# huggingface/diffusers

Measured on AMD Instinct MI355X. Metric: images/sec @ SDXL-base 1024x1024 50-step EulerDiscrete CFG bf16, higher is better.
Workload: dtype bf16; 1 GPU; SDXL-base-1.0 U-Net (2567 M params) x 50 EulerDiscrete steps, CFG 5.0 (batch 2), 128x128 latents + AutoencoderKL decode to 1024x1024; 1 prompt per GPU; global_batch=1, parallelism=dp1 (independent prompts, replicas), denoise_steps=50, output_type=pt, hip_graph=True, output_finite=True, rccl_ranks=1, tuned_live=0, cpu_binding=none

## Files before the change

### diffusers_amd/_lib.py

```python
from __future__ import annotations

import ctypes as C
import threading
from pathlib import Path

_PKG = Path(__file__).resolve().parent
LIB_PATH = _PKG / "_C" / "libdiffusers_amd.so"

DA_OK = 0
ERRORS = {1: "DA_ERR_INVALID", 2: "DA_ERR_LAUNCH", 3: "DA_ERR_UNSUPPORTED"}
ACT_NONE, ACT_GEGLU, ACT_GELU_TANH, ACT_SILU, ACT_GELU_ERF, ACT_QUICK_GELU, ACT_GEGLU_TANH = 0, 1, 2, 3, 4, 5, 6
ACT_RELU = 7
(TILE_AUTO, TILE_128x128, TILE_64x128, TILE_128x64, TILE_64x64, TILE_256x128, TILE_128x256, TILE_256x256,
 TILE_128x128_W8, TILE_K2_128x128, TILE_K2_128x80, TILE_K2_128x160, TILE_K2_80x128, TILE_K2_128x64,
 TILE_K1_128x320, TILE_K1_256x128, TILE_K1_128x256, TILE_K1_256x160, TILE_K1_256x256, TILE_K1_256x320,
 TILE_K3_256x256, TILE_K3_256x320) = range(22)
TILE_NAMES = ("auto", "128x128", "64x128", "128x64", "64x64", "256x128", "128x256", "256x256", "128x128w8",
              "k2:128x128", "k2:128x80", "k2:128x160", "k2:80x128", "k2:128x64",
              "k1:128x320", "k1:256x128", "k1:128x256", "k1:256x160", "k1:256x256", "k1:256x320",
              "k3:256x256", "k3:256x320")
FIRST_K2_TILE = TILE_K2_128x128
STAGE_REGISTER, STAGE_LDS_DIRECT, STAGE_LDS_DIRECT3, STAGE_LDS_DIRECT4, STAGE_LDS_DIRECT6, STAGE_LDS_DIRECT8 = range(6)
STAGE_PINGPONG, STAGE_PINGPONG3 = 6, 7
RING_SLOTS = (2, 2, 3, 4, 6, 8)
# ... 14 lines not shown
        ("M", C.c_int), ("N", C.c_int), ("K", C.c_int),
        ("lda", C.c_int), ("ldw", C.c_int), ("ldc", C.c_int), ("ldr", C.c_int), ("ld_rowvec", C.c_int),
        ("ld_gate", C.c_int),
        ("rows_per_batch", C.c_int),
        ("alpha", C.c_float), ("out_scale", C.c_float),
        ("act", C.c_int), ("out_f32", C.c_int), ("conv", C.c_int),
        ("Hin", C.c_int), ("Win", C.c_int), ("C1", C.c_int), ("C2", C.c_int),
        ("Hout", C.c_int), ("Wout", C.c_int), ("stride", C.c_int), ("up", C.c_int), ("pad", C.c_int),
        ("tile", C.c_int), ("staging", C.c_int), ("gate_f32", C.c_int),
        ("split_k", C.c_int), ("workspace", C.c_void_p), ("sync_flags", C.c_void_p), ("workspace_bytes", C.c_longlong),
        ("stats_out", C.c_void_p), ("stats_ld", C.c_int), ("ln_stats", C.c_void_p), ("ln_stats_ld", C.c_int),
        ("ln_parts", C.c_int), ("ln_s", C.c_void_p), ("ln_c", C.c_void_p), ("ln_eps", C.c_float), ("k_valid", C.c_int),
        ("prefetch", C.c_void_p), ("prefetch_bytes", C.c_longlong),
        ("vt", C.c_void_p), ("vt_col0", C.c_int), ("ld_vt", C.c_longlong),
        ("xa_k", C.c_void_p), ("xa_vt", C.c_void_p), ("xa_skv", C.c_int), ("xa_skv_alloc", C.c_int), ("xa_k_ld", C.c_int),
        ("xa_vt_ld", C.c_longlong), ("xa_scale", C.c_float),
    ]


class AttentionParams(C.Structure):
    _fields_ = [
        ("q", C.c_void_p), ("k", C.c_void_p), ("vt", C.c_void_p), ("out", C.c_void_p),
        ("B", C.c_int), ("H", C.c_int), ("Sq", C.c_int), ("Skv", C.c_int), ("Skv_alloc", C.c_int), ("D", C.c_int),
        ("q_batch_stride", C.c_longlong), ("k_batch_stride", C.c_longlong),
        ("vt_batch_stride", C.c_longlong), ("o_batch_stride", C.c_longlong),
        ("q_row_stride", C.c_int), ("k_row_stride", C.c_int), ("vt_ld", C.c_int), ("o_row_stride", C.c_int),
        ("scale", C.c_float), ("ring_slots", C.c_int),
        ("bias", C.c_void_p), ("bias_batch_stride", C.c_longlong), ("bias_head_stride", C.c_longlong),
        ("bias_row_stride", C.c_int), ("bias_f32", C.c_int), ("causal", C.c_int), ("q_block", C.c_int), ("pv_delay", C.c_int),
        ("algo", C.c_int),
        ("split_ws", C.c_void_p), ("split_ws_bytes", C.c_longlong), ("kv_split", C.c_int),
# ... 138 lines not shown
```

### diffusers_amd/autoencoder_kl.py

```python
from __future__ import annotations

from dataclasses import dataclass
from typing import Dict, Optional

import torch

from . import ops
from .config_utils import check_to
from .loading import PretrainedMixin
from . import _lib as L
from .layers import Downsample2D, GroupNorm, ResnetBlock2D, Upsample2D, Weights
from .unet_2d_condition import FrozenConfig

bf16 = torch.bfloat16


@dataclass
class DecoderOutput:
    sample: torch.Tensor


_DEFAULTS = dict(
    in_channels=3, out_channels=3, down_block_types=("DownEncoderBlock2D",), up_block_types=("UpDecoderBlock2D",),
    block_out_channels=(64,), layers_per_block=1, act_fn="silu", latent_channels=4, norm_num_groups=32, sample_size=32,
# ... 239 lines not shown
        self.conv_in_w = ops.pack_conv_weight(ci)
        self.conv_in_b = w.get("decoder.conv_in.bias")

        self.mid_res0 = ResnetBlock2D(w, "decoder.mid_block.resnets.0", groups, eps)
        self.mid_attn = VaeAttention(w, "decoder.mid_block.attentions.0", groups, eps) \
            if c.mid_block_add_attention else None
        self.mid_res1 = ResnetBlock2D(w, "decoder.mid_block.resnets.1", groups, eps)

        self.up = []
        n = len(boc)
        for i in range(n):
            pre = f"decoder.up_blocks.{i}"
            stage = {"resnets": [ResnetBlock2D(w, f"{pre}.resnets.{j}", groups, eps)
                                 for j in range(c.layers_per_block + 1)], "up": None}
            if i != n - 1:
                stage["up"] = Upsample2D(w, f"{pre}.upsamplers.0")
            self.up.append(stage)
        self.conv_norm_out = GroupNorm(w, "decoder.conv_norm_out", groups, eps)
        self.conv_out_w = ops.pack_conv_weight(w.get("decoder.conv_out.weight"))
        self.conv_out_b = w.get("decoder.conv_out.bias")
        self.encoder = _Encoder(w, c, groups, eps) if w.has("encoder.conv_in.weight") else None
        if strict:
            extra = [k for k in w.unused() if k.startswith(("decoder.", "post_quant_conv.", "encoder.", "quant_conv."))]
            if extra:
                raise RuntimeError(f"unexpected VAE keys: {extra[:8]}")
        self._built = True
        return self

    def to(self, *args, **kwargs):
        return check_to(self, args, kwargs)

# ... 58 lines not shown
```

### diffusers_amd/csrc/gemm.hip

```cpp
#include "gemm_kernel.cuh"
#include "gemm2_shared.cuh"

namespace da_gemm {
int dispatch_conv(const da_gemm_params& p, int tile, int staging, hipStream_t s);
}
namespace da_gemm2 {
int dispatch_lin(const da_gemm_params& p, int tile, int staging, hipStream_t s);
int dispatch_conv(const da_gemm_params& p, int tile, int staging, hipStream_t s);
}
namespace da_gemm3 {
int dispatch_lin(const da_gemm_params& p, int tile, int staging, hipStream_t s);
}
namespace da_c64 {
int launch(const da_gemm_params& p, hipStream_t s);
}

namespace {

struct TileShape {
  int bm, bn, waves;
};
constexpr TileShape kTiles[] = {{0, 0, 0},      {128, 128, 4}, {64, 128, 4},  {128, 64, 4}, {64, 64, 4},
                                {256, 128, 8},  {128, 256, 8}, {256, 256, 8}, {128, 128, 8},
                                {128, 128, 8},  {128, 80, 8},  {128, 160, 8}, {80, 128, 8}, {128, 64, 8},
                                {128, 320, 8},  {256, 128, 8}, {128, 256, 8}, {256, 160, 8}, {256, 256, 8}, {256, 320, 8},
                                {256, 256, 8},  {256, 320, 8}};
static_assert(sizeof(kTiles) / sizeof(kTiles[0]) == DA_TILE_COUNT, "kTiles / DA_TILE_* mismatch");
inline bool is_k3(int tile) { return tile == DA_TILE_K3_256x256 || tile == DA_TILE_K3_256x320; }
inline bool is_k2(int tile) { return tile >= DA_TILE_K2_128x128 && !is_k3(tile); }
constexpr int kNumTiles = sizeof(kTiles) / sizeof(kTiles[0]);

int pick_tile(const da_gemm_params& p) {
  auto nblk = [&](int t) {
    return (long)((p.M + kTiles[t].bm - 1) / kTiles[t].bm) * ((p.N + kTiles[t].bn - 1) / kTiles[t].bn);
  };
  const bool geglu = (p.act == DA_ACT_GEGLU || p.act == DA_ACT_GEGLU_TANH);
  const bool narrow = !geglu && ((p.N & 127) != 0) && ((p.N % 128) <= 64);
  if (narrow) return (nblk(DA_TILE_128x64) >= 200) ? DA_TILE_128x64 : DA_TILE_64x64;
  if (nblk(DA_TILE_256x128) >= 480) return DA_TILE_256x128;
  if (nblk(DA_TILE_128x128) >= 128) return DA_TILE_128x128;
  if (nblk(DA_TILE_64x128) >= 128 || geglu) return DA_TILE_64x128;
  return DA_TILE_64x64;
}

int validate_conv(const da_gemm_params& p) {
  if (p.C1 <= 0 || (p.C1 & 63) || (p.C2 & 63) || p.C2 < 0) return DA_ERR_UNSUPPORTED;
  if (p.conv != 1 && p.conv != 3) return DA_ERR_UNSUPPORTED;
  if (p.K != p.conv * p.conv * (p.C1 + p.C2)) return DA_ERR_INVALID;
  if (p.stride != 1 && p.stride != 2) return DA_ERR_UNSUPPORTED;
  if (p.up != 0 && p.up != 1) return DA_ERR_INVALID;
  if (p.Hin <= 0 || p.Win <= 0 || p.Hout <= 0 || p.Wout <= 0) return DA_ERR_INVALID;
  if (p.M % (p.Hout * p.Wout)) return DA_ERR_INVALID;
  return DA_OK;
}

int validate(da_gemm_params& p) {
  if (p.M <= 0 || p.N <= 0 || p.K <= 0) return DA_ERR_INVALID;
  if ((p.K & 63) || (p.N & 3) || (p.ldc & 3)) return DA_ERR_UNSUPPORTED;
  if (!p.A || !p.W || !p.C) return DA_ERR_INVALID;
  if (p.residual && (p.ldr & 3)) return DA_ERR_UNSUPPORTED;
  if (p.rowvec && (p.rows_per_batch <= 0 || (p.ld_rowvec & 3))) return DA_ERR_INVALID;
  if (p.gate && (p.rows_per_batch <= 0 || (p.ld_gate & 3))) return DA_ERR_INVALID;
  if (p.gate_f32 < 0 || p.gate_f32 > 2) return DA_ERR_INVALID;
  if (p.alpha == 0.0f) p.alpha = 1.0f;
  if (p.out_scale == 0.0f) p.out_scale = 1.0f;
  if (p.conv) {
    const int v = validate_conv(p);
    if (v != DA_OK) return v;
    if (p.C2 > 0 && !p.A2) return DA_ERR_INVALID;
  } else {
    if ((p.lda & 7) || (p.ldw & 7)) return DA_ERR_UNSUPPORTED;
  }
  if ((p.act == DA_ACT_GEGLU || p.act == DA_ACT_GEGLU_TANH) &&
      ((p.N & 127) || p.out_f32 || p.residual || p.rowvec || p.gate || p.bias_rows))
    return DA_ERR_UNSUPPORTED;
  if (p.act < 0 || p.act > DA_ACT_RELU) return DA_ERR_INVALID;
  if (p.gate && p.gate_f32 == 2 && p.conv == 3) return DA_ERR_UNSUPPORTED;
  if (p.split_k < 0 || p.split_k > DA_SPLITK_MAX) return DA_ERR_INVALID;
  if (p.split_k > 1 && (p.stats_out || p.ln_stats)) return DA_ERR_UNSUPPORTED;
  if (p.k_valid < 0 || (p.k_valid > 0 && (p.k_valid > (p.conv ? p.C1 : p.K) || (p.conv && p.C2 != 0)))) return DA_ERR_INVALID;
// ... 4 lines not shown
    return DA_ERR_INVALID;
  return DA_OK;
}

int stats_parts(const da_gemm_params& p, int tile) {
  if (is_k2(tile)) {
    const int band = (tile == DA_TILE_K2_128x80 || tile == DA_TILE_K2_128x160) ? 80 : 0;
    return band ? (p.N + band - 1) / band : 0;
  }
  return (p.N + kTiles[tile].bn - 1) / kTiles[tile].bn;
}

bool tile_ok(const da_gemm_params& p, int tile) {
  if (tile <= 0 || tile >= kNumTiles) return false;
  if (p.act == DA_ACT_RELU) return false;
  if (p.gate && p.gate_f32 == 2 && (is_k2(tile) || is_k3(tile))) return false;
  if (is_k3(tile)) {
    if (p.conv || p.split_k > 1 || p.stats_out || (p.ln_stats && tile != DA_TILE_K3_256x320) || p.vt || p.xa_k) return false;
    if (tile == DA_TILE_K3_256x320)
      return (p.act == DA_ACT_GEGLU || p.act == DA_ACT_GEGLU_TANH) && (p.M % 256) == 0 && (p.N % 320) == 0 && !(p.ldc & 7) &&
             !((size_t)p.C & 15);
    return true;
  }
  if (is_k2(tile)) {
    const bool geglu = (p.act == DA_ACT_GEGLU || p.act == DA_ACT_GEGLU_TANH);
    const bool geglu_ok = tile == DA_TILE_K2_128x128 || tile == DA_TILE_K1_256x128 || tile == DA_TILE_K1_128x256 ||
                          tile == DA_TILE_K1_256x256 || tile == DA_TILE_K1_256x320 || (tile == DA_TILE_K1_128x320 && !p.conv);
    const bool lnf_lin = tile == DA_TILE_K2_128x80 || tile == DA_TILE_K2_128x160;
    const bool lnf_cons = lnf_lin || tile == DA_TILE_K1_128x256 || tile == DA_TILE_K1_256x128;
    if (p.xa_k) return !p.conv && p.split_k <= 1 && !geglu && !p.stats_out && !p.vt && tile == DA_TILE_K2_128x128;
// ... 160 lines not shown
```

### diffusers_amd/csrc/gemm2_kernel.cuh

```cuda
#pragma once
#include <cstdlib>
#include <type_traits>

#include "common.cuh"
#include "diffusers_amd.h"
#include "gemm2_shared.cuh"

namespace da_gemm2 {


#if defined(DA_GEMM2_TRACE)
__device__ unsigned long long* g_da2_trace;
#define DA2_TRACE(i) tr_[i] = __builtin_readcyclecounter()
#else
#define DA2_TRACE(i) ((void)0)
#endif



template <int KG, int WM, int WN, int MT, int NT, int NSLOT, bool CONV, bool PP = false, bool STREAMW = false, bool GIL = false,
          bool LNF = false, int XA = 0>
__global__ __launch_bounds__(512) void igemm2_bf16_kernel(const da_gemm_params p, const int xcd_gx_chunk) {
#if defined(__HIP_DEVICE_COMPILE__)
  const int xcd_gx = xcd_gx_chunk & 255;
  static_assert((KG == 1 || KG == 2) && KG * WM * WN == 8, "eight waves: one or two K-groups");
  constexpr int BM = 16 * MT * WM, BN = 16 * NT * WN;
  constexpr int PX = BM / 8, PW = BN / 8;
  constexpr int XBYTES = BM * 128, SLICE = (BM + BN) * 128, PAIR = KG * SLICE;
  static_assert(!PP || KG == 2, "ping-pong is a property of the two K-groups");
  static_assert(!STREAMW || (KG == 1 && NSLOT == 2 && !CONV), "streaming-W loop: one K-group, two-slice ring, nn.Linear");
  static_assert(!GIL || (KG == 1 && !CONV && WN == 2 && (NT % 2) == 0), "GEGLU-interleaved ownership: two wave columns, value / gate tile pairs");
  static_assert(!LNF || (!CONV && !STREAMW), "LayerNorm fold: nn.Linear instantiations of the ring loops");
  static_assert(XA == 0 || (LNF && KG == 2 && WM == 2 && WN == 2 && MT == 4 && NT == 4 && NSLOT == 2 && XA <= 8),
                "cross-attention epilogue: the 128 x 128 two-K-group tile (a wave finishes 32 rows x one 64-wide head)");
  constexpr int SW = PP ? 4 : 8;
  constexpr int UX = PP ? PX : KG * PX, UW = PP ? PW : KG * PW;
  constexpr int XI = (UX + SW - 1) / SW, WI = (UW + SW - 1) / SW;
  constexpr int XRAG = UX % SW ? 1 : 0, WRAG = UW % SW ? 1 : 0;
  static_assert(NSLOT == 2 || NSLOT == 3, "ring of 2 or 3 slice pairs");
  constexpr int DUMP = 1024;
  constexpr int LNSC = LNF ? 2 * BN * 4 : 0;
  constexpr int XA_K_OFF = 4 * MT * NT * 1024, XA_KB = XA * 16 * 128, XA_V_OFF = XA_K_OFF + 32768;
  static_assert(XA == 0 || (2 * XA_KB <= 32768 && XA_V_OFF + 32768 <= NSLOT * PAIR), "cross-attention operands do not fit the ring");
  static_assert(NSLOT * PAIR + DUMP + LNSC <= 160 * 1024, "LDS ring exceeds the 160 KiB of a CU");
  static_assert(BM % 8 == 0 && BN % 8 == 0, "tile rows are staged in 8-row pieces");
  static_assert(!CONV || (UX % SW) == 0, "conv: the slice of an activation piece must be a compile-time constant");
  static_assert((NSLOT - 1) * (XI + WI) <= 63, "vmcnt is a 6-bit counter");
// ... 2 lines not shown

#if defined(DA_GEMM2_TRACE)
  unsigned long long tr_[8] = {0, 0, 0, 0, 0, 0, 0, 0};
#endif
  DA2_TRACE(0);
  const int t = threadIdx.x;
  const int lane = t & 63, wave = __builtin_amdgcn_readfirstlane(t >> 6);
  const int g = KG == 2 ? wave >> 2 : 0, wq = KG == 2 ? wave & 3 : wave;
  const int wm = wq / WN, wn = wq - wm * WN;
  const int r16 = lane & 15, kq = lane >> 4;

  const int tiles_n = (p.N + BN - 1) / BN, tiles_m = (p.M + BM - 1) / BM;
  const int gyn = 8 / xcd_gx;
  const int tm_per = (tiles_m + gyn - 1) / gyn, tn_per = (tiles_n + xcd_gx - 1) / xcd_gx;
  const int bid = (int)blockIdx.x;
  const int xcd = bid & 7, kblk = bid >> 3;
  const int gy = xcd / xcd_gx, gx = xcd - gy * xcd_gx;
  const int lm = kblk / tn_per, ln = kblk - lm * tn_per;
  const int tm = gy * tm_per + lm, tn = gx * tn_per + ln;
  if (tm >= tiles_m || tn >= tiles_n) return;
  const int m0 = tm * BM, n0 = tn * BN;

  const uint16_t* __restrict__ A = (const uint16_t*)p.A;
  const uint16_t* __restrict__ A2 = (const uint16_t*)p.A2;
  const uint16_t* __restrict__ Wt = (const uint16_t*)p.W;
  const int nk = p.K >> 6;
  const int nk2 = (nk + KG - 1) / KG;
  const int Ctot = CONV ? (p.C1 + p.C2) : 0;
  const int Hv = CONV ? (p.Hin << p.up) : 0, Wv = CONV ? (p.Win << p.up) : 0;

  int x_h[XI], x_r[XI], w_h[WI], w_r[WI];
// ... 16 lines not shown
  }
  const int own_half = PP ? g * SLICE : 0;
  constexpr int my_loads = XI + WI;

  int xr_base[XI], xr_oy[XI], xr_ox[XI];
  if constexpr (CONV) {
    const int hw = p.Hout * p.Wout;
#pragma unroll
    for (int i = 0; i < XI; ++i) {
      const int m = m0 + x_r[i] * 8 + (lane >> 3);
      if (m < p.M) {
        const int b = m / hw;
        const int rem = m - b * hw;
        const int oy = rem / p.Wout;
        xr_base[i] = b * p.Hin;
        xr_oy[i] = oy * p.stride - p.pad;
        xr_ox[i] = (rem - oy * p.Wout) * p.stride - p.pad;
      } else {
        xr_base[i] = 0;
        xr_oy[i] = -100000;
        xr_ox[i] = -100000;
      }
    }
  }

  size_t xbase = 0, xbytes = 0x7fffffff, x2bytes = 0x7fffffff;
  int pb = 0;
  if constexpr (CONV) {
    const int hw = p.Hout * p.Wout;
    const int b0 = m0 / hw;
    const int oy0 = (m0 - b0 * hw) / p.Wout;
    pb = __builtin_amdgcn_readfirstlane((b0 * p.Hin + (max(0, oy0 * p.stride - p.pad) >> p.up)) * p.Win);
    const size_t pix_left = (size_t)(p.M / hw) * p.Hin * p.Win - (size_t)pb;
    xbytes = min(pix_left * p.C1 * 2, (size_t)0x7fffffff);
    x2bytes = min(pix_left * p.C2 * 2, (size_t)0x7fffffff);
  } else {
    xbase = (size_t)m0 * p.lda;
  }
  __amdgpu_buffer_rsrc_t rs_x = uniform_rsrc(A + (CONV ? (size_t)pb * p.C1 : xbase), xbytes);
  __amdgpu_buffer_rsrc_t rs_x2 = uniform_rsrc((CONV && A2) ? A2 + (size_t)pb * p.C2 : A, x2bytes);
  __amdgpu_buffer_rsrc_t rs_w = uniform_rsrc(Wt + (size_t)n0 * p.ldw, 0x7fffffff);

  int vo_x[XI], vo_x2[XI], vo_w[WI];
#pragma unroll
  for (int i = 0; i < XI; ++i) {
    const int row = x_r[i] * 8 + (lane >> 3);
    const int sc = (lane & 7) ^ ((row >> 1) & 7);
    if constexpr (!CONV) vo_x[i] = (min(row, p.M - 1 - m0) * p.lda + sc * 8) * 2;
    else vo_x[i] = 0;
    vo_x2[i] = 0;
  }
#pragma unroll
  for (int i = 0; i < WI; ++i) {
    const int row = w_r[i] * 8 + (lane >> 3);
    const int sc = (lane & 7) ^ ((row >> 1) & 7);
    vo_w[i] = (min(row, p.N - 1 - n0) * p.ldw + sc * 8) * 2;
// ... 98 lines not shown
        st_s[h] = want;
      }
    }
    st_zero[0] = (KG * st_pr + (PP ? g : 0) < nk) ? 0 : (int)0x80000000;
    st_zero[1] = (KG * st_pr + 1 < nk) ? 0 : (int)0x80000000;
  };
#define DA2_WAIT_PAIRS(PAIRS) asm volatile("s_waitcnt vmcnt(%0)" ::"n"((PAIRS) * my_loads) : "memory")

  constexpr bool SPLIT_M = KG == 1 || (MT % 2) == 0;
  static_assert(SPLIT_M || (NT % 2) == 0, "one of the wave tile's dimensions must split between the two K-groups");
  constexpr int MH = (KG == 2 && SPLIT_M) ? MT / 2 : MT, NH = (KG == 1 || SPLIT_M) ? NT : NT / 2;
  const bool geglu = (p.act == DA_ACT_GEGLU || p.act == DA_ACT_GEGLU_TANH);
  auto row_of = [&](int ih) { return m0 + (wm * MT + (SPLIT_M ? g * MH : 0) + ih) * 16 + r16; };
  auto col_tile = [&](int jh) { return GIL ? 4 * (jh >> 1) + 2 * (jh & 1) + wn : wn * NT + (SPLIT_M ? 0 : g * NH) + jh; };
  auto col_of = [&](int jh) { return n0 + col_tile(jh) * 16 + 4 * kq; };
  constexpr bool PF = MH * NH <= (CONV ? 8 : 12);
  constexpr bool STG = NH >= 2;
  constexpr int PPR = 2 * NH, NPIECE = 16 * PPR, TT = (NPIECE + 63) / 64, ROWB = NH * 64 + 32;
  static_assert(!STG || (KG == 2 ? 4 * MT * NT * 1024 : 0) + 8 * 16 * ROWB <= NSLOT * PAIR, "output staging does not fit the ring");
  constexpr int STATS_OFF = (KG == 2 ? 4 * MT * NT * 1024 : 0) + 8 * 16 * ROWB;
  static_assert(!(LNF && STG) || STATS_OFF + 8 * TT * 64 * 8 <= NSLOT * PAIR, "statistics scratch does not fit the ring");
  const bool wide = STG && !GIL && !geglu && !p.out_f32 && !(p.ldc & 7) && !((size_t)p.C & 15) && !(p.N & 7) &&
                    (!p.residual || (!(p.ldr & 7) && !((size_t)p.residual & 15)));
  const int band_col0 = n0 + (wn * NT + (SPLIT_M ? 0 : g * NH)) * 16;
  auto band_row0 = [&](int ih) { return m0 + (wm * MT + (SPLIT_M ? g * MH : 0) + ih) * 16; };
  constexpr bool PFN = PF && !STG;
  uint2 res_v[PFN ? MH : 1][PFN ? NH : 1], bias_v[NH], rowvec_v[PF ? MH : 1][PF ? NH : 1];
  uint4 resw[(PF && STG) ? MH : 1][(PF && STG) ? TT : 1];
#pragma unroll
  for (int ih = 0; ih < (PF ? MH : 1); ++ih)
// ... 627 lines not shown
          uint4 pk;
          if constexpr (PACKED) {
            pk = *(const uint4*)(stg + row * (ROWB / 2) + c8 * 16);
          } else {
            const float4 lo = *(const float4*)(stg + row * ROWB + c8 * 32), hi = *(const float4*)(stg + row * ROWB + c8 * 32 + 16);
            float o[8] = {lo.x, lo.y, lo.z, lo.w, hi.x, hi.y, hi.z, hi.w};
            uint4 rw = make_uint4(DA_NEG0_BF2, DA_NEG0_BF2, DA_NEG0_BF2, DA_NEG0_BF2);
            if constexpr (PF) rw = resw[ih][t];
            else if (has_res && inside) rw = *(const uint4*)(resid + (size_t)mo * p.ldr + no);
            o[0] += bf_lo(rw.x); o[1] += bf_hi(rw.x); o[2] += bf_lo(rw.y); o[3] += bf_hi(rw.y);
            o[4] += bf_lo(rw.z); o[5] += bf_hi(rw.z); o[6] += bf_lo(rw.w); o[7] += bf_hi(rw.w);
#pragma unroll
            for (int e = 0; e < 8; ++e) o[e] *= p.out_scale;
            pk.x = pack_bf2(o[0], o[1]); pk.y = pack_bf2(o[2], o[3]); pk.z = pack_bf2(o[4], o[5]); pk.w = pack_bf2(o[6], o[7]);
          }
          if (inside) *(uint4*)((uint16_t*)p.C + (size_t)mo * p.ldc + no) = pk;
          if constexpr (LNF) {
            if (p.stats_out) {
              float r[8];
              unpack8(pk, r);
              const float s1 = ((r[0] + r[1]) + (r[2] + r[3])) + ((r[4] + r[5]) + (r[6] + r[7]));
              const float s2 = ((r[0] * r[0] + r[1] * r[1]) + (r[2] * r[2] + r[3] * r[3])) +
                               ((r[4] * r[4] + r[5] * r[5]) + (r[6] * r[6] + r[7] * r[7]));
              part[q] = inside ? make_float2(s1, s2) : make_float2(0.f, 0.f);
            }
          }
        }
        if constexpr (LNF) {
          if (p.stats_out) {
            asm volatile("s_waitcnt lgkmcnt(0)" ::: "memory");
            if (lane < 16) {
// ... 25 lines not shown
#pragma unroll
      for (int jh = 0; jh < NH; ++jh) {
        const int n = col_of(jh);
        if (n >= p.N) continue;
        float o[4];
#pragma unroll
        for (int e = 0; e < 4; ++e) o[e] = keep[ih][jh][e] * p.alpha;
        ln_apply4(o, ih, n);
        uint2 rvv = make_uint2(0, 0), rsv = make_uint2(DA_NEG0_BF2, DA_NEG0_BF2);
        if constexpr (PF) rvv = rowvec_v[ih][jh];
        else if (has_rowvec) rvv = *(const uint2*)((const uint16_t*)p.rowvec + (size_t)bidx * p.ld_rowvec + n);
        if constexpr (PFN) rsv = res_v[ih][jh];
        else if (has_res) rsv = *(const uint2*)((const uint16_t*)p.residual + (size_t)m * p.ldr + n);
        epilogue4<ACT, GATE, true>(p, o, n, bidx, brow, bias_v[jh], rvv, rsv);
        if (p.out_f32) {
          *(float4*)((float*)p.C + (size_t)m * p.ldc + n) = make_float4(o[0], o[1], o[2], o[3]);
        } else {
          uint2 pk;
          pk.x = pack_bf2(o[0], o[1]);
          pk.y = pack_bf2(o[2], o[3]);
          *(uint2*)((uint16_t*)p.C + (size_t)m * p.ldc + n) = pk;
        }
      }
    }
  };
  if constexpr (LNF && !GIL) {
    if (p.vt && n0 >= p.vt_col0) {
      uint16_t* __restrict__ vt = (uint16_t*)p.vt;
#pragma unroll
      for (int ih = 0; ih < MH; ++ih) {
        const int m = row_of(ih);
#pragma unroll
        for (int jh = 0; jh < NH; ++jh) {
          const int n = col_of(jh);
          if (n >= p.N) continue;
          float o[4];
// ... 38 lines not shown
    }
  }
  DA2_TRACE_END();
#undef DA2_TRACE_END
#undef DA2_LDS
#undef DA2_WAIT_PAIRS
#undef DA2_SG_DS
#undef DA2_SG_MF
#undef DA2_SG_VM
#endif
}



template <int KG, int WM, int WN, int MT, int NT, int NSLOT, bool CONV, bool PP = false, bool STREAMW = false, bool GIL = false,
          bool LNF = false, int XA = 0>
int launch(const da_gemm_params& p, hipStream_t s) {
  constexpr int BM = 16 * MT * WM, BN = 16 * NT * WN;
  const LaunchGeom geom = launch_geom(p, BM, BN, CONV);
  constexpr size_t lds = (size_t)NSLOT * KG * (BM + BN) * 128 + 1024 + (LNF ? 2 * BN * 4 : 0);
  auto kern = igemm2_bf16_kernel<KG, WM, WN, MT, NT, NSLOT, CONV, PP, STREAMW, GIL, LNF, XA>;
  static bool attr_set = false;
  if (!attr_set) {
    if (hipFuncSetAttribute((const void*)kern, hipFuncAttributeMaxDynamicSharedMemorySize, (int)lds) != hipSuccess)
      return DA_ERR_LAUNCH;
    attr_set = true;
  }
  DA_LAUNCH(kern, dim3(geom.grid), dim3(512), lds, s, p, geom.gx | (CONV ? conv_chunk_slices(p, geom.rows_xcd) << 8 : 0));
  DA_CHECK_LAUNCH();
  return DA_OK;
}

inline int stats_band_cols(int tile) { return (tile == DA_TILE_K2_128x80 || tile == DA_TILE_K2_128x160) ? 80 : 0; }

inline int dispatch_lnf(const da_gemm_params& p, int tile, int staging, hipStream_t s) {
  const bool geglu = (p.act == DA_ACT_GEGLU || p.act == DA_ACT_GEGLU_TANH);
  const int ns = (staging == DA_STAGE_LDS_DIRECT || staging == DA_STAGE_PINGPONG) ? 2
                 : (staging == DA_STAGE_LDS_DIRECT3 || staging == DA_STAGE_PINGPONG3) ? 3 : 0;
  const bool pp = staging == DA_STAGE_PINGPONG || staging == DA_STAGE_PINGPONG3;
  if (ns == 0) return DA_ERR_UNSUPPORTED;
  if (p.xa_k) {
    if (tile != DA_TILE_K2_128x128 || ns != 2 || geglu || !p.xa_vt || p.vt || p.stats_out || p.residual || p.gate || p.rowvec ||
        p.bias_rows || p.out_f32 || p.act != DA_ACT_NONE || p.out_scale != 1.0f || (p.N & 127) || (p.ldc & 7) ||
// ... 39 lines not shown
    case DA_TILE_K1_256x128:
      if (geglu || p.stats_out || pp) break;
      return ns == 2 ? launch<1, 4, 2, 4, 4, 2, false, false, false, false, true>(p, s)
                     : launch<1, 4, 2, 4, 4, 3, false, false, false, false, true>(p, s);
  }
  return DA_ERR_UNSUPPORTED;
}

template <bool CONV>
int dispatch(const da_gemm_params& p, int tile, int staging, hipStream_t s) {
  if (p.split_k > 1 || !staging_fits(p)) return DA_ERR_UNSUPPORTED;
  if (p.stats_out || p.ln_stats || p.vt || p.xa_k) {
    if constexpr (CONV) return DA_ERR_UNSUPPORTED;
    else return dispatch_lnf(p, tile, staging, s);
  }
  const bool geglu = (p.act == DA_ACT_GEGLU || p.act == DA_ACT_GEGLU_TANH);
  if (geglu && tile != DA_TILE_K2_128x128 && tile != DA_TILE_K1_256x128 && tile != DA_TILE_K1_128x256 && tile != DA_TILE_K1_256x256 &&
      tile != DA_TILE_K1_256x320 && tile != DA_TILE_K1_128x320)
    return DA_ERR_UNSUPPORTED;
  const int ns = (staging == DA_STAGE_LDS_DIRECT || staging == DA_STAGE_PINGPONG) ? 2
                 : (staging == DA_STAGE_LDS_DIRECT3 || staging == DA_STAGE_PINGPONG3) ? 3 : 0;
  if (ns == 0) return DA_ERR_UNSUPPORTED;
  if (staging == DA_STAGE_PINGPONG || staging == DA_STAGE_PINGPONG3) {
    switch (tile) {
      case DA_TILE_K2_128x128:
        if (ns == 2) return launch<2, 2, 2, 4, 4, 2, CONV, true>(p, s);
        break;
      case DA_TILE_K2_128x80:
        return ns == 2 ? launch<2, 4, 1, 2, 5, 2, CONV, true>(p, s) : launch<2, 4, 1, 2, 5, 3, CONV, true>(p, s);
      case DA_TILE_K2_128x160:
// ... 58 lines not shown
```

### diffusers_amd/layers.py

```python
from __future__ import annotations

import os
from typing import Dict, Optional

import torch

from . import _lib as L
from . import ops

bf16 = torch.bfloat16


class Weights:

    def __init__(self, state_dict: Dict[str, torch.Tensor], device):
        self.sd = state_dict
        self.device = torch.device(device)
        self.used = set()

    def has(self, name: str) -> bool:
        return name in self.sd

    def get(self, name: str) -> torch.Tensor:
        if name not in self.sd:
# ... 146 lines not shown

    def __init__(self, w: Weights, prefix: str, padding: int = 1):
        if padding not in (0, 1):
            raise ValueError("Downsample2D: padding must be 0 or 1")
        self.conv = Conv3x3(w, prefix + ".conv")
        self.padding = padding

    def __call__(self, x):
        if self.padding == 1:
            return self.conv(x, stride=2)
        return self.conv(x, stride=2, pad=0, pad_after=1)


class Upsample2D:

    def __init__(self, w: Weights, prefix: str):
        self.conv = Conv3x3(w, prefix + ".conv")

    def __call__(self, x):
        return self.conv(x, up=True)


class CrossKV:

    __slots__ = ("k", "vt", "skv", "skv_alloc", "batch", "bias", "buf")

    def __init__(self, k, vt, skv, skv_alloc, batch, bias=None, buf=None):
        self.k, self.vt, self.skv, self.skv_alloc, self.batch = k, vt, skv, skv_alloc, batch
        self.buf = buf
        self.bias = bias


KERNEL_HEAD_DIMS = (64, 96, 128, 160)

# ... 241 lines not shown
```

### diffusers_amd/loading.py

```python
from __future__ import annotations

import hashlib
import itertools
import json
import os
import warnings
from collections.abc import Mapping
from pathlib import Path
from typing import Dict, Iterator, List, Optional

import torch

from . import packed_cache

CONFIG_NAME = "config.json"
WEIGHTS_NAME = "diffusion_pytorch_model"
PACKED_DIR = "diffusers_amd_packed"


class LazyCheckpoint(Mapping):

    def __init__(self, files: List[Path], device: str = "cpu"):
        from safetensors import safe_open
        self._files = [Path(f) for f in files]
# ... 179 lines not shown
    @classmethod
    def from_pretrained(cls, pretrained_model_name_or_path, subfolder: Optional[str] = None, torch_dtype=None,
                        variant: Optional[str] = None, device="cuda", use_safetensors: Optional[bool] = None,
                        cache_packed: bool = True, cache_dir: Optional[os.PathLike] = None, **config_overrides):
        if torch_dtype not in (None, torch.bfloat16):
            raise ValueError(f"{cls.__name__}.from_pretrained: torch_dtype={torch_dtype} -- the HIP engine computes in bfloat16")
        if use_safetensors is False:
            raise ValueError(f"{cls.__name__}.from_pretrained: pickle checkpoints are not read; use safetensors")
        from .config_utils import from_reference_config
        d = _resolve_dir(pretrained_model_name_or_path, subfolder)
        files = _weight_files(d, variant)
        cfg = read_config(d)
        cfg.update(config_overrides)
        from . import ops
        fp = checkpoint_fingerprint(files, extra=cls.__name__ + json.dumps(cfg, sort_keys=True, default=str)
                                    + (f"+lnfold{int(ops.LN_FOLD)}qkv" if ops.LN_FOLD else "") + "+tembcat")
        cdir = Path(cache_dir) if cache_dir is not None else d / PACKED_DIR
        cfile = cdir / f"{cls.__name__}-{fp}.safetensors"
        model = None
        if cache_packed and cfile.exists():
            try:
                model = packed_cache.load_packed(cls, cfile, device=device, expect_fingerprint=fp)
            except ValueError:
                model = None
        if model is None:
            model = from_reference_config(cls, cfg)
            model.load_state_dict(LazyCheckpoint(files), device=device)
            if cache_packed:
                try:
                    packed_cache.save_packed(model, cfile, source_fingerprint=fp)
                except OSError:
# ... 57 lines not shown
```

### diffusers_amd/ops.py

```python
from __future__ import annotations

import ctypes as C
import os
import threading
import weakref
from typing import Optional

import torch

from . import _lib as L
from . import tuning

bf16 = torch.bfloat16

DEFAULT_STAGING = L.STAGE_LDS_DIRECT
DEFAULT_TILE = L.TILE_AUTO
TUNING = True

PREFETCH = os.environ.get("DIFFUSERS_AMD_PREFETCH", "1") != "0"
_prefetch_tls = threading.local()


class WeightPrefetch:
    def __init__(self, models=(), owner=None, slots=()):
# ... 516 lines not shown
    p.conv = ksize
    p.Hin, p.Win, p.C1, p.C2, p.Hout, p.Wout = H, W_, C1, C2, Hout, Wout
    p.stride, p.up, p.pad = stride, int(up), pad
    return p


def conv_chunk_channels(x: torch.Tensor, w: torch.Tensor, tile: int, *, ksize: int = 3, x2: Optional[torch.Tensor] = None,
                        stride: int = 1, up: bool = False, pad: Optional[int] = None, pad_after: int = 0) -> int:
    p = _conv_params(x, w, ksize, x2, stride, up, pad, pad_after)
    r = int(L.load().da_conv_chunk_channels(C.byref(p), int(tile)))
    if r < 0:
        L.check(-r, f"da_conv_chunk_channels(tile {L.TILE_NAMES[tile] if 0 <= tile < len(L.TILE_NAMES) else tile})")
    return r


def linear_small_m(x: torch.Tensor, w: torch.Tensor, bias: Optional[torch.Tensor] = None, *, act_in: int = L.ACT_NONE,
                   act_out: int = L.ACT_NONE, residual: Optional[torch.Tensor] = None,
                   out: Optional[torch.Tensor] = None) -> torch.Tensor:
    _req(x, "x"), _req(w, "w")
    M, K = x.shape
    N = w.shape[0]
    if w.shape[1] != K or not w.is_contiguous():
        raise ValueError("linear_small_m: weight must be contiguous [N][K]")
    if out is None:
        out = torch.empty((M, N), device=x.device, dtype=bf16)
    L.check(L.load().da_linear_small_m_bf16(
        x.data_ptr(), w.data_ptr(), _ptr(bias), _ptr(residual), out.data_ptr(), M, N, K, _rows2d(x, "x"),
        _rows2d(out, "out"), _rows2d(residual, "residual") if residual is not None else 0, act_in, act_out, _stream()),
        "da_linear_small_m_bf16")
    return out
# ... 745 lines not shown
```

### diffusers_amd/tuning.py

```python
from __future__ import annotations

import atexit
import ctypes as C
import json
import os
from pathlib import Path
from typing import Dict, Optional, Tuple

import torch

from . import _lib as L

_PKG = Path(__file__).resolve().parent
DB_PATH = Path(os.environ.get("DIFFUSERS_AMD_TUNE_DB", _PKG / "tuned" / "gfx950.json"))
LIVE = os.environ.get("DIFFUSERS_AMD_TUNE", "1") != "0"
ITERS = 3
FLUSH_BYTES = 320 << 20

_table: Dict[str, Tuple[int, int, float, int]] = {}
LIVE_COUNT = 0
_loaded = False
_dirty = False
_scratch = {}
_session_tuned = set()


def _m_key(m: int) -> int:
    if m <= (1 << 20):
        return m
    sh = m.bit_length() - 3
    return (m >> sh) << sh


def key_of(p: "L.GemmParams") -> str:
    kv = f":v{p.k_valid}" if p.k_valid else ""
    if p.conv:
        return (f"conv{p.conv}:M{_m_key(int(p.M))}:N{p.N}:C{p.C1}+{p.C2}:H{p.Hin}x{p.Win}:s{p.stride}:u{p.up}:a{p.act}"
                f":r{int(bool(p.residual))}{kv}")
    return f"lin:M{_m_key(int(p.M))}:N{p.N}:K{p.K}:a{p.act}:f{p.out_f32}:r{int(bool(p.residual))}{kv}"


def _load() -> None:
    global _loaded
    _loaded = True
    if DB_PATH.exists():
        try:
            raw = json.loads(DB_PATH.read_text())
            for k, v in raw.get("entries", {}).items():
                _table[k] = (int(v[0]), int(v[1]), float(v[2]), int(v[3]) if len(v) > 3 else 1)
        except (ValueError, KeyError, TypeError) as e:
            raise RuntimeError(f"diffusers_amd: unreadable tuning table {DB_PATH}: {e}") from e


# ... 95 lines not shown
```

### diffusers_amd/unet_2d_condition.py

```python
from __future__ import annotations

from dataclasses import dataclass
from typing import Any, Dict, List, Optional

import torch

from . import ops
from .config_utils import check_to
from .loading import PretrainedMixin
from .layers import (GroupNorm, ResnetBlock2D, TimeProjections, TimestepEmbedding, Transformer2DModel, Upsample2D, Weights,
                     encoder_mask_bias, pad_encoder_states)
from .unet_blocks import build_down_blocks, build_mid_block, walk_down, walk_mid

bf16 = torch.bfloat16


@dataclass
class UNet2DConditionOutput:
    sample: torch.Tensor


class FrozenConfig(dict):
    def __getattr__(self, k):
        try:
# ... 98 lines not shown
        self.mid = build_mid_block(w, c)

        rheads = tuple(reversed(heads))
        rlpb = tuple(reversed(lpb))
        rtlpb = tuple(reversed(tlpb)) if c.reverse_transformer_layers_per_block is None \
            else _tup(c.reverse_transformer_layers_per_block, n)
        self.up = []
        for i, btype in enumerate(c.up_block_types):
            pre = f"up_blocks.{i}"
            stage = {"resnets": [], "attns": [], "up": None}
            for j in range(rlpb[i] + 1):
                stage["resnets"].append(ResnetBlock2D(w, f"{pre}.resnets.{j}", groups, eps))
                if btype == "CrossAttnUpBlock2D":
                    stage["attns"].append(Transformer2DModel(w, f"{pre}.attentions.{j}", rheads[i], rtlpb[i], groups))
            if i != n - 1:
                stage["up"] = Upsample2D(w, f"{pre}.upsamplers.0")
            self.up.append(stage)
        self.time_proj = TimeProjections([r for st in self.down for r in st["resnets"]] + self.mid["resnets"] +
                                         [r for st in self.up for r in st["resnets"]])

        self.conv_norm_out = GroupNorm(w, "conv_norm_out", groups, eps)
        self.conv_out_w = ops.pack_conv_weight(w.get("conv_out.weight"))
        self.conv_out_b = w.get("conv_out.bias")
        if strict and w.unused():
            raise RuntimeError(f"unexpected keys in state_dict: {w.unused()[:8]} ...")
        self._temb_dim = temb_dim
        self._built = True
        return self

    def to(self, *args, **kwargs):
        return check_to(self, args, kwargs)
# ... 209 lines not shown
```

### include/diffusers_amd.h

```cpp
#ifndef DIFFUSERS_AMD_H
#define DIFFUSERS_AMD_H

#include <stddef.h>
#include <stdint.h>

#ifdef __cplusplus
extern "C" {
#endif

#define DA_OK 0
#define DA_ERR_INVALID 1
#define DA_ERR_LAUNCH 2
#define DA_ERR_UNSUPPORTED 3

#define DA_ACT_NONE 0
#define DA_ACT_GEGLU 1
#define DA_ACT_GELU_TANH 2
#define DA_ACT_SILU 3
#define DA_ACT_GELU_ERF 4
#define DA_ACT_QUICK_GELU 5
#define DA_ACT_GEGLU_TANH 6
#define DA_ACT_RELU 7

#define DA_TILE_AUTO 0
// ... 73 lines not shown
  int ln_stats_ld, ln_parts;
  const float* ln_s;
  const float* ln_c;
  float ln_eps;
  int k_valid;
  const void* prefetch;
  long long prefetch_bytes;
  void* vt;
  int vt_col0;
  long long ld_vt;
  const void* xa_k;
  const void* xa_vt;
  int xa_skv, xa_skv_alloc, xa_k_ld;
  long long xa_vt_ld;
  float xa_scale;
} da_gemm_params;

int da_gemm_stats_parts(const da_gemm_params* p);

int da_conv_chunk_channels(const da_gemm_params* p, int tile);

#define DA_LN_MAX_PARTS 64
#define DA_LN_PAIR_LOADS 6
#define DA_SPLITK_FLAGS 4096
#define DA_SPLITK_MAX 24
#define DA_SPLITK_ERR_SLOT (DA_SPLITK_FLAGS - 1)

int da_gemm_bf16(const da_gemm_params* p, void* stream);

int da_gemm_pair_bf16(const da_gemm_params* a, const da_gemm_params* b, void* stream);
// ... 175 lines not shown
```

Baseline: 1.001 images/s.

## Replace nearest-2x upsample + 3x3 conv with four-phase sub-pixel 2x2 conv GEMM

Folds nearest-neighbour 2x upsampling followed by a 3x3 conv into four 2x2 phase convolutions on the un-upsampled input. Each phase's weights are precomputed by summing taps, and each phase's output is written interleaved into the 2x output. This cuts the conv's K from 9C to 4C per output pixel and removes the upsampled-input reads. It applies to the U-Net upsamplers (the VAE is opted out) and adds a phase mode to the conv GEMM kernel with a restricted tile set. The packed weight cache key changes.

```diff
diff --git a/diffusers_amd/_lib.py b/diffusers_amd/_lib.py
--- a/diffusers_amd/_lib.py
+++ b/diffusers_amd/_lib.py
@@ -52,7 +52,7 @@
         ("prefetch", C.c_void_p), ("prefetch_bytes", C.c_longlong),
         ("vt", C.c_void_p), ("vt_col0", C.c_int), ("ld_vt", C.c_longlong),
         ("xa_k", C.c_void_p), ("xa_vt", C.c_void_p), ("xa_skv", C.c_int), ("xa_skv_alloc", C.c_int), ("xa_k_ld", C.c_int),
-        ("xa_vt_ld", C.c_longlong), ("xa_scale", C.c_float),
+        ("xa_vt_ld", C.c_longlong), ("xa_scale", C.c_float), ("phase", C.c_int),
     ]
 
 
diff --git a/diffusers_amd/autoencoder_kl.py b/diffusers_amd/autoencoder_kl.py
--- a/diffusers_amd/autoencoder_kl.py
+++ b/diffusers_amd/autoencoder_kl.py
@@ -277,7 +277,7 @@
             stage = {"resnets": [ResnetBlock2D(w, f"{pre}.resnets.{j}", groups, eps)
                                  for j in range(c.layers_per_block + 1)], "up": None}
             if i != n - 1:
-                stage["up"] = Upsample2D(w, f"{pre}.upsamplers.0")
+                stage["up"] = Upsample2D(w, f"{pre}.upsamplers.0", subpixel=False)
             self.up.append(stage)
         self.conv_norm_out = GroupNorm(w, "decoder.conv_norm_out", groups, eps)
         self.conv_out_w = ops.pack_conv_weight(w.get("decoder.conv_out.weight"))
diff --git a/diffusers_amd/csrc/gemm.hip b/diffusers_amd/csrc/gemm.hip
--- a/diffusers_amd/csrc/gemm.hip
+++ b/diffusers_amd/csrc/gemm.hip
@@ -31,6 +31,7 @@
 constexpr int kNumTiles = sizeof(kTiles) / sizeof(kTiles[0]);
 
 int pick_tile(const da_gemm_params& p) {
+  if (p.phase) return DA_TILE_K1_128x320;
   auto nblk = [&](int t) {
     return (long)((p.M + kTiles[t].bm - 1) / kTiles[t].bm) * ((p.N + kTiles[t].bn - 1) / kTiles[t].bn);
   };
@@ -45,7 +46,12 @@
 
 int validate_conv(const da_gemm_params& p) {
   if (p.C1 <= 0 || (p.C1 & 63) || (p.C2 & 63) || p.C2 < 0) return DA_ERR_UNSUPPORTED;
-  if (p.conv != 1 && p.conv != 3) return DA_ERR_UNSUPPORTED;
+  if (p.phase) {
+    if (p.phase != 1) return DA_ERR_INVALID;
+    if (p.conv != 2 || p.stride != 1 || p.up != 0 || p.C2 != 0 || p.Hout != p.Hin || p.Wout != p.Win) return DA_ERR_INVALID;
+  } else if (p.conv != 1 && p.conv != 3) {
+    return DA_ERR_UNSUPPORTED;
+  }
   if (p.K != p.conv * p.conv * (p.C1 + p.C2)) return DA_ERR_INVALID;
   if (p.stride != 1 && p.stride != 2) return DA_ERR_UNSUPPORTED;
   if (p.up != 0 && p.up != 1) return DA_ERR_INVALID;
@@ -64,6 +70,9 @@
   if (p.gate_f32 < 0 || p.gate_f32 > 2) return DA_ERR_INVALID;
   if (p.alpha == 0.0f) p.alpha = 1.0f;
   if (p.out_scale == 0.0f) p.out_scale = 1.0f;
+  if (p.phase && (!p.conv || p.residual || p.rowvec || p.gate || p.bias_rows || p.stats_out || p.ln_stats || p.vt || p.xa_k ||
+                  p.k_valid || p.split_k > 1 || p.act != DA_ACT_NONE || (long long)p.M * 4 > 0x7fffffffll))
+    return p.conv ? DA_ERR_UNSUPPORTED : DA_ERR_INVALID;
   if (p.conv) {
     const int v = validate_conv(p);
     if (v != DA_OK) return v;
@@ -98,6 +107,7 @@
 bool tile_ok(const da_gemm_params& p, int tile) {
   if (tile <= 0 || tile >= kNumTiles) return false;
   if (p.act == DA_ACT_RELU) return false;
+  if (p.phase) return tile == DA_TILE_K1_256x160 || tile == DA_TILE_K1_128x320;
   if (p.gate && p.gate_f32 == 2 && (is_k2(tile) || is_k3(tile))) return false;
   if (is_k3(tile)) {
     if (p.conv || p.split_k > 1 || p.stats_out || (p.ln_stats && tile != DA_TILE_K3_256x320) || p.vt || p.xa_k) return false;
diff --git a/diffusers_amd/csrc/gemm2_kernel.cuh b/diffusers_amd/csrc/gemm2_kernel.cuh
--- a/diffusers_amd/csrc/gemm2_kernel.cuh
+++ b/diffusers_amd/csrc/gemm2_kernel.cuh
@@ -19,7 +19,7 @@
 
 
 template <int KG, int WM, int WN, int MT, int NT, int NSLOT, bool CONV, bool PP = false, bool STREAMW = false, bool GIL = false,
-          bool LNF = false, int XA = 0>
+          bool LNF = false, int XA = 0, bool PH = false>
 __global__ __launch_bounds__(512) void igemm2_bf16_kernel(const da_gemm_params p, const int xcd_gx_chunk) {
 #if defined(__HIP_DEVICE_COMPILE__)
   const int xcd_gx = xcd_gx_chunk & 255;
@@ -31,6 +31,7 @@
   static_assert(!STREAMW || (KG == 1 && NSLOT == 2 && !CONV), "streaming-W loop: one K-group, two-slice ring, nn.Linear");
   static_assert(!GIL || (KG == 1 && !CONV && WN == 2 && (NT % 2) == 0), "GEGLU-interleaved ownership: two wave columns, value / gate tile pairs");
   static_assert(!LNF || (!CONV && !STREAMW), "LayerNorm fold: nn.Linear instantiations of the ring loops");
+  static_assert(!PH || (CONV && KG == 1), "phase mode: the one-K-group conv tiles");
   static_assert(XA == 0 || (LNF && KG == 2 && WM == 2 && WN == 2 && MT == 4 && NT == 4 && NSLOT == 2 && XA <= 8),
                 "cross-attention epilogue: the 128 x 128 two-K-group tile (a wave finishes 32 rows x one 64-wide head)");
   constexpr int SW = PP ? 4 : 8;
@@ -63,7 +64,9 @@
   const int gyn = 8 / xcd_gx;
   const int tm_per = (tiles_m + gyn - 1) / gyn, tn_per = (tiles_n + xcd_gx - 1) / xcd_gx;
   const int bid = (int)blockIdx.x;
-  const int xcd = bid & 7, kblk = bid >> 3;
+  const int xcd = bid & 7, kblk = PH ? bid >> 5 : bid >> 3;
+  const int ph = PH ? (bid >> 3) & 3 : 0;
+  const int pad_y = PH ? 1 - (ph >> 1) : p.pad, pad_x = PH ? 1 - (ph & 1) : p.pad;
   const int gy = xcd / xcd_gx, gx = xcd - gy * xcd_gx;
   const int lm = kblk / tn_per, ln = kblk - lm * tn_per;
   const int tm = gy * tm_per + lm, tn = gx * tn_per + ln;
@@ -110,8 +113,8 @@
         const int rem = m - b * hw;
         const int oy = rem / p.Wout;
         xr_base[i] = b * p.Hin;
-        xr_oy[i] = oy * p.stride - p.pad;
-        xr_ox[i] = (rem - oy * p.Wout) * p.stride - p.pad;
+        xr_oy[i] = oy * p.stride - pad_y;
+        xr_ox[i] = (rem - oy * p.Wout) * p.stride - pad_x;
       } else {
         xr_base[i] = 0;
         xr_oy[i] = -100000;
@@ -126,7 +129,7 @@
     const int hw = p.Hout * p.Wout;
     const int b0 = m0 / hw;
     const int oy0 = (m0 - b0 * hw) / p.Wout;
-    pb = __builtin_amdgcn_readfirstlane((b0 * p.Hin + (max(0, oy0 * p.stride - p.pad) >> p.up)) * p.Win);
+    pb = __builtin_amdgcn_readfirstlane((b0 * p.Hin + (max(0, oy0 * p.stride - pad_y) >> p.up)) * p.Win);
     const size_t pix_left = (size_t)(p.M / hw) * p.Hin * p.Win - (size_t)pb;
     xbytes = min(pix_left * p.C1 * 2, (size_t)0x7fffffff);
     x2bytes = min(pix_left * p.C2 * 2, (size_t)0x7fffffff);
@@ -135,7 +138,7 @@
   }
   __amdgpu_buffer_rsrc_t rs_x = uniform_rsrc(A + (CONV ? (size_t)pb * p.C1 : xbase), xbytes);
   __amdgpu_buffer_rsrc_t rs_x2 = uniform_rsrc((CONV && A2) ? A2 + (size_t)pb * p.C2 : A, x2bytes);
-  __amdgpu_buffer_rsrc_t rs_w = uniform_rsrc(Wt + (size_t)n0 * p.ldw, 0x7fffffff);
+  __amdgpu_buffer_rsrc_t rs_w = uniform_rsrc(Wt + ((PH ? (size_t)ph * p.N : (size_t)0) + n0) * p.ldw, 0x7fffffff);
 
   int vo_x[XI], vo_x2[XI], vo_w[WI];
 #pragma unroll
@@ -264,6 +267,14 @@
   auto row_of = [&](int ih) { return m0 + (wm * MT + (SPLIT_M ? g * MH : 0) + ih) * 16 + r16; };
   auto col_tile = [&](int jh) { return GIL ? 4 * (jh >> 1) + 2 * (jh & 1) + wn : wn * NT + (SPLIT_M ? 0 : g * NH) + jh; };
   auto col_of = [&](int jh) { return n0 + col_tile(jh) * 16 + 4 * kq; };
+  auto out_row = [&](int m) -> size_t {
+    if constexpr (PH) {
+      const int hw = p.Hin * p.Win, b = m / hw, rem = m - b * hw, i = rem / p.Win;
+      return ((size_t)(b * 2 * p.Hin + 2 * i + (ph >> 1)) * (2 * p.Win) + 2 * (rem - i * p.Win) + (ph & 1));
+    } else {
+      return (size_t)m;
+    }
+  };
   constexpr bool PF = MH * NH <= (CONV ? 8 : 12);
   constexpr bool STG = NH >= 2;
   constexpr int PPR = 2 * NH, NPIECE = 16 * PPR, TT = (NPIECE + 63) / 64, ROWB = NH * 64 + 32;
@@ -921,7 +932,7 @@
             for (int e = 0; e < 8; ++e) o[e] *= p.out_scale;
             pk.x = pack_bf2(o[0], o[1]); pk.y = pack_bf2(o[2], o[3]); pk.z = pack_bf2(o[4], o[5]); pk.w = pack_bf2(o[6], o[7]);
           }
-          if (inside) *(uint4*)((uint16_t*)p.C + (size_t)mo * p.ldc + no) = pk;
+          if (inside) *(uint4*)((uint16_t*)p.C + out_row(mo) * p.ldc + no) = pk;
           if constexpr (LNF) {
             if (p.stats_out) {
               float r[8];
@@ -977,12 +988,12 @@
         else if (has_res) rsv = *(const uint2*)((const uint16_t*)p.residual + (size_t)m * p.ldr + n);
         epilogue4<ACT, GATE, true>(p, o, n, bidx, brow, bias_v[jh], rvv, rsv);
         if (p.out_f32) {
-          *(float4*)((float*)p.C + (size_t)m * p.ldc + n) = make_float4(o[0], o[1], o[2], o[3]);
+          *(float4*)((float*)p.C + out_row(m) * p.ldc + n) = make_float4(o[0], o[1], o[2], o[3]);
         } else {
           uint2 pk;
           pk.x = pack_bf2(o[0], o[1]);
           pk.y = pack_bf2(o[2], o[3]);
-          *(uint2*)((uint16_t*)p.C + (size_t)m * p.ldc + n) = pk;
+          *(uint2*)((uint16_t*)p.C + out_row(m) * p.ldc + n) = pk;
         }
       }
     }
@@ -1051,19 +1062,19 @@
 
 
 template <int KG, int WM, int WN, int MT, int NT, int NSLOT, bool CONV, bool PP = false, bool STREAMW = false, bool GIL = false,
-          bool LNF = false, int XA = 0>
+          bool LNF = false, int XA = 0, bool PH = false>
 int launch(const da_gemm_params& p, hipStream_t s) {
   constexpr int BM = 16 * MT * WM, BN = 16 * NT * WN;
   const LaunchGeom geom = launch_geom(p, BM, BN, CONV);
   constexpr size_t lds = (size_t)NSLOT * KG * (BM + BN) * 128 + 1024 + (LNF ? 2 * BN * 4 : 0);
-  auto kern = igemm2_bf16_kernel<KG, WM, WN, MT, NT, NSLOT, CONV, PP, STREAMW, GIL, LNF, XA>;
+  auto kern = igemm2_bf16_kernel<KG, WM, WN, MT, NT, NSLOT, CONV, PP, STREAMW, GIL, LNF, XA, PH>;
   static bool attr_set = false;
   if (!attr_set) {
     if (hipFuncSetAttribute((const void*)kern, hipFuncAttributeMaxDynamicSharedMemorySize, (int)lds) != hipSuccess)
       return DA_ERR_LAUNCH;
     attr_set = true;
   }
-  DA_LAUNCH(kern, dim3(geom.grid), dim3(512), lds, s, p, geom.gx | (CONV ? conv_chunk_slices(p, geom.rows_xcd) << 8 : 0));
+  DA_LAUNCH(kern, dim3(PH ? 4 * geom.grid : geom.grid), dim3(512), lds, s, p, geom.gx | (CONV ? conv_chunk_slices(p, geom.rows_xcd) << 8 : 0));
   DA_CHECK_LAUNCH();
   return DA_OK;
 }
@@ -1133,6 +1144,14 @@
     if constexpr (CONV) return DA_ERR_UNSUPPORTED;
     else return dispatch_lnf(p, tile, staging, s);
   }
+  if (p.phase) {
+    if constexpr (CONV) {
+      if (staging != DA_STAGE_LDS_DIRECT) return DA_ERR_UNSUPPORTED;
+      if (tile == DA_TILE_K1_128x320) return launch<1, 4, 2, 2, 10, 2, true, false, false, false, false, 0, true>(p, s);
+      if (tile == DA_TILE_K1_256x160) return launch<1, 4, 2, 4, 5, 2, true, false, false, false, false, 0, true>(p, s);
+    }
+    return DA_ERR_UNSUPPORTED;
+  }
   const bool geglu = (p.act == DA_ACT_GEGLU || p.act == DA_ACT_GEGLU_TANH);
   if (geglu && tile != DA_TILE_K2_128x128 && tile != DA_TILE_K1_256x128 && tile != DA_TILE_K1_128x256 && tile != DA_TILE_K1_256x256 &&
       tile != DA_TILE_K1_256x320 && tile != DA_TILE_K1_128x320)
diff --git a/diffusers_amd/layers.py b/diffusers_amd/layers.py
--- a/diffusers_amd/layers.py
+++ b/diffusers_amd/layers.py
@@ -184,10 +184,18 @@
 
 class Upsample2D:
 
-    def __init__(self, w: Weights, prefix: str):
-        self.conv = Conv3x3(w, prefix + ".conv")
+    def __init__(self, w: Weights, prefix: str, subpixel: bool = True, pixels: int = 0):
+        shape = tuple(w.sd[prefix + ".conv.weight"].shape) if w.has(prefix + ".conv.weight") else (1, 1)
+        self.subpixel = bool(subpixel and ops.UP_SUBPIXEL and pixels >= ops.UP2X_MIN_PIXELS and shape[1] % 64 == 0 and shape[0] % ops.UP2X_COLS == 0)
+        if self.subpixel:
+            self.weight = ops.pack_conv_up2x_weight(w.get(prefix + ".conv.weight"))
+            self.bias = w.opt(prefix + ".conv.bias")
+        else:
+            self.conv = Conv3x3(w, prefix + ".conv")
 
     def __call__(self, x):
+        if self.subpixel:
+            return ops.conv2d_up2x_nhwc(x, self.weight, self.bias)
         return self.conv(x, up=True)
 
 
diff --git a/diffusers_amd/loading.py b/diffusers_amd/loading.py
--- a/diffusers_amd/loading.py
+++ b/diffusers_amd/loading.py
@@ -217,7 +217,8 @@
         cfg.update(config_overrides)
         from . import ops
         fp = checkpoint_fingerprint(files, extra=cls.__name__ + json.dumps(cfg, sort_keys=True, default=str)
-                                    + (f"+lnfold{int(ops.LN_FOLD)}qkv" if ops.LN_FOLD else "") + "+tembcat")
+                                    + (f"+lnfold{int(ops.LN_FOLD)}qkv" if ops.LN_FOLD else "") + "+tembcat"
+                                    + ("+up2x" if ops.UP_SUBPIXEL else ""))
         cdir = Path(cache_dir) if cache_dir is not None else d / PACKED_DIR
         cfile = cdir / f"{cls.__name__}-{fp}.safetensors"
         model = None
diff --git a/diffusers_amd/ops.py b/diffusers_amd/ops.py
--- a/diffusers_amd/ops.py
+++ b/diffusers_amd/ops.py
@@ -554,6 +554,73 @@
     return r
 
 
+UP2X_TAPS = (((0,), (1, 2)), ((0, 1), (2,)))
+UP_SUBPIXEL = os.environ.get("DIFFUSERS_AMD_UP_SUBPIXEL", "1") == "1"
+UP2X_TILES = (L.TILE_K1_256x160, L.TILE_K1_128x320)
+UP2X_MIN_PIXELS = 1024
+UP2X_COLS = 160
+
+
+def up2x_phase_weights(w: torch.Tensor) -> torch.Tensor:
+    wf = w if w.dtype == torch.float64 else w.float()
+
+    def taps(t, dim, ks):
+        r = t.select(dim, ks[0])
+        for k in ks[1:]:
+            r = r + t.select(dim, k)
+        return r
+    rows = [taps(wf, 2, UP2X_TAPS[py][dy]) for py in (0, 1) for dy in (0, 1)]
+    out = wf.new_empty((2, 2) + tuple(w.shape[:2]) + (2, 2))
+    for py in (0, 1):
+        for dy in (0, 1):
+            r = rows[2 * py + dy]
+            for px in (0, 1):
+                for dx in (0, 1):
+                    out[py, px, :, :, dy, dx] = taps(r, 2, UP2X_TAPS[px][dx])
+    return out
+
+
+def pack_conv_up2x_weight(w: torch.Tensor) -> torch.Tensor:
+    n, c = w.shape[:2]
+    if tuple(w.shape[2:]) != (3, 3):
+        raise ValueError(f"pack_conv_up2x_weight: expected a [N][C][3][3] weight, got {tuple(w.shape)}")
+    ph = up2x_phase_weights(w)
+    return ph.permute(0, 1, 2, 4, 5, 3).reshape(4, n, 4 * c).to(w.dtype).contiguous()
+
+
+def conv2d_up2x_nhwc(x: torch.Tensor, w4: torch.Tensor, bias: Optional[torch.Tensor] = None, *, tile: Optional[int] = None,
+                     out: Optional[torch.Tensor] = None) -> torch.Tensor:
+    _req(x, "x"), _req(w4, "w4")
+    B, H, W_, C1 = x.shape
+    if w4.dim() != 3 or w4.shape[0] != 4 or w4.shape[2] != 4 * C1 or not w4.is_contiguous() or not x.is_contiguous():
+        raise ValueError(f"conv2d_up2x_nhwc: x {tuple(x.shape)} / w4 {tuple(w4.shape)}: expected contiguous [B][H][W][C] and [4][N][4C]")
+    N = w4.shape[1]
+    if out is None:
+        out = torch.empty((B, 2 * H, 2 * W_, N), device=x.device, dtype=bf16)
+    else:
+        _req(out, "out")
+        if tuple(out.shape) != (B, 2 * H, 2 * W_, N) or not out.is_contiguous():
+            raise ValueError("conv2d_up2x_nhwc: out must be contiguous [B][2H][2W][N]")
+    p = L.GemmParams()
+    p.M, p.N, p.K = B * H * W_, N, 4 * C1
+    p.lda, p.ldw, p.ldc = 0, 4 * C1, N
+    p.conv, p.phase = 2, 1
+    p.Hin, p.Win, p.C1, p.C2, p.Hout, p.Wout = H, W_, C1, 0, H, W_
+    p.stride, p.up, p.pad = 1, 0, 1
+    p.A, p.W, p.C, p.bias = x.data_ptr(), w4.data_ptr(), out.data_ptr(), _ptr(bias)
+    p.alpha, p.out_scale, p.act, p.split_k = 1.0, 1.0, L.ACT_NONE, 1
+    _prefetch_hook(p, x, w4)
+    ent = tuning.table().get(tuning.key_of(p)) if TUNING and tile is None else None
+    p._auto = ent is not None
+    if ent is not None:
+        p.tile, p.staging = ent[0], ent[1]
+    else:
+        p.tile = tile if tile is not None else (L.TILE_K1_256x160 if p.M % 256 == 0 and N % 160 == 0 else L.TILE_K1_128x320)
+        p.staging = L.STAGE_LDS_DIRECT
+    _launch_gemm(p, _stream(), "da_gemm_bf16(conv, up2x phases)")
+    return out
+
+
 def linear_small_m(x: torch.Tensor, w: torch.Tensor, bias: Optional[torch.Tensor] = None, *, act_in: int = L.ACT_NONE,
                    act_out: int = L.ACT_NONE, residual: Optional[torch.Tensor] = None,
                    out: Optional[torch.Tensor] = None) -> torch.Tensor:
diff --git a/diffusers_amd/tuning.py b/diffusers_amd/tuning.py
--- a/diffusers_amd/tuning.py
+++ b/diffusers_amd/tuning.py
@@ -35,8 +35,9 @@
 def key_of(p: "L.GemmParams") -> str:
     kv = f":v{p.k_valid}" if p.k_valid else ""
     if p.conv:
+        ph = ":ph" if p.phase else ""
         return (f"conv{p.conv}:M{_m_key(int(p.M))}:N{p.N}:C{p.C1}+{p.C2}:H{p.Hin}x{p.Win}:s{p.stride}:u{p.up}:a{p.act}"
-                f":r{int(bool(p.residual))}{kv}")
+                f":r{int(bool(p.residual))}{kv}{ph}")
     return f"lin:M{_m_key(int(p.M))}:N{p.N}:K{p.K}:a{p.act}:f{p.out_f32}:r{int(bool(p.residual))}{kv}"
 
 
diff --git a/diffusers_amd/unet_2d_condition.py b/diffusers_amd/unet_2d_condition.py
--- a/diffusers_amd/unet_2d_condition.py
+++ b/diffusers_amd/unet_2d_condition.py
@@ -136,7 +136,8 @@
                 if btype == "CrossAttnUpBlock2D":
                     stage["attns"].append(Transformer2DModel(w, f"{pre}.attentions.{j}", rheads[i], rtlpb[i], groups))
             if i != n - 1:
-                stage["up"] = Upsample2D(w, f"{pre}.upsamplers.0")
+                side = c.sample_size[0] if isinstance(c.sample_size, (tuple, list)) else c.sample_size
+                stage["up"] = Upsample2D(w, f"{pre}.upsamplers.0", pixels=(int(side) >> (n - 1 - i)) ** 2 if side else 0)
             self.up.append(stage)
         self.time_proj = TimeProjections([r for st in self.down for r in st["resnets"]] + self.mid["resnets"] +
                                          [r for st in self.up for r in st["resnets"]])
diff --git a/include/diffusers_amd.h b/include/diffusers_amd.h
--- a/include/diffusers_amd.h
+++ b/include/diffusers_amd.h
@@ -111,6 +111,7 @@
   int xa_skv, xa_skv_alloc, xa_k_ld;
   long long xa_vt_ld;
   float xa_scale;
+  int phase;
 } da_gemm_params;
 
 int da_gemm_stats_parts(const da_gemm_params* p);
```

New measurement: 1.010 images/s (median of 6 runs). No clear change (+0.9%).
